# google-research/semivl

Measured on AMD Instinct MI355X. Metric: train images/sec (512^2, ViT-B/16), higher is better.
Workload: dtype f32 (fp32 in / out / accumulate everywhere; the MFMA products as split 16-bit terms with fp32 accumulation: the ViT's linears, in_proj weight gradients and fused attention and the decoder's 3x3 convolutions (tiled: forward, input and weight gradient; dilated: forward, input gradient) on fp16 x 2 ope; 1 GPU; SemiVL step, pascal N=21, vlm-vlg-aspp-s2p4-sk04-ftap-mcvitb, 512x512, bs=16/GPU labeled + 16/GPU unlabeled (BASELINE configs[1]); global_batch=32, parallelism=dp1

## Files before the change

### semivl_amd/csrc/gemm_planes_impl.h

```cpp
#pragma once
#include "svl_common.h"
#include "planes_split_h2.h"
#include <atomic>
#include <type_traits>

struct PlanesP {
  const char* A;
  const char* B;
  long a_ks, b_ks;
  const int* a_se;
  const int* b_se;
  const float* a_rn;
  const float* b_bd;
  int* p_se;
  int p_np;
  int epi_fast;
  int b_rb;
  int M, N, K;
  float* C;
  long ldc;
  char* P;
  long p_ks;
  const float* bias;
  int act;
  float* preact;
  const float* resid;
  long ldr;
  int accumulate;
  int tiles_n, full_m, tail_rows;
  int rcnt[8], fstart[8];
  int panel;
#ifdef SVL_X6P_TIMING
  unsigned long long* dbg;
#endif
};
#ifdef SVL_X6P_TIMING
#define X6P_STAMP(slot)                                                                      \
  do {                                                                                       \
    if (p.dbg && lane == 0 && (wave & 3) == 0) {                                             \
      p.dbg[((long)blockIdx.x * 2 + (wave >> 2)) * 8 + (slot)] = wall_clock64();            \
      p.dbg[((long)blockIdx.x * 2 + (wave >> 2)) * 8 + 4 + (slot)] = clock64();             \
    }                                                                                        \
  } while (0)
#else
#define X6P_STAMP(slot) do {} while (0)
#endif

namespace {

typedef __bf16 bf16x8 __attribute__((ext_vector_type(8)));
typedef int i32x4 __attribute__((ext_vector_type(4)));
typedef unsigned int u32x4 __attribute__((ext_vector_type(4)));

constexpr int BM = 256;
constexpr int CH = 1024;
constexpr int NSTAGE = 3;

template <int I, int N_, typename F>
__device__ __forceinline__ void static_for(F&& f) {
  if constexpr (I < N_) {
    f(std::integral_constant<int, I>{});
    static_for<I + 1, N_>(f);
  }
}

template <int NP> struct FragOf;
template <> struct FragOf<3> { typedef bf16x8 T; };
template <> struct FragOf<2> { typedef f16x8 T; };
template <int NP>
__device__ __forceinline__ f32x16 mfma16(const typename FragOf<NP>::T& x, const typename FragOf<NP>::T& y, const f32x16& c) {
  if constexpr (NP == 3) return __builtin_amdgcn_mfma_f32_32x32x16_bf16(x, y, c, 0, 0, 0);
  else return __builtin_amdgcn_mfma_f32_32x32x16_f16(x, y, c, 0, 0, 0);
}


__device__ __forceinline__ void glds16(const char* base_, unsigned lane_off, unsigned lds_dst_) {
  const unsigned long long bv = (unsigned long long)base_;
  const unsigned b_hi = (unsigned)__builtin_amdgcn_readfirstlane((int)(bv >> 32));
  const unsigned b_lo = (unsigned)__builtin_amdgcn_readfirstlane((int)(unsigned)bv);
  const char* base = (const char*)(((unsigned long long)b_hi << 32) | (unsigned long long)b_lo);
  const unsigned lds_dst = __builtin_amdgcn_readfirstlane(lds_dst_);
  unsigned keep;
  asm volatile("s_mov_b32 %0, m0\n\ts_mov_b32 m0, %3\n\ts_nop 3\n\tglobal_load_lds_dwordx4 %2, %1\n\ts_mov_b32 m0, %0"
               : "=&s"(keep)
               : "s"(base), "v"(lane_off), "s"(lds_dst)
               : "memory");
}

template <int N_>
__device__ __forceinline__ void wait_vm() {
  static_assert(N_ >= 0 && N_ < 64, "vmcnt");
  asm volatile("s_waitcnt vmcnt(%0)" ::"n"(N_) : "memory");
}

__device__ __forceinline__ void split3x8(const float (&x)[8], bf16x8& h0, bf16x8& h1, bf16x8& h2) {
#pragma unroll
  for (int j = 0; j < 8; ++j) {
    float v = x[j];
    h0[j] = (__bf16)v;
    v -= (float)h0[j];
    h1[j] = (__bf16)v;
    v -= (float)h1[j];
    h2[j] = (__bf16)v;
  }
}


struct TileRef { int m0, rows, tn; };
__device__ __forceinline__ TileRef tile_of_block(const PlanesP& p) {
  TileRef t;
  const int lin = (int)blockIdx.x, x = lin & 7, idx = lin >> 3;
  const int rc = p.rcnt[x];
  if (idx < rc) {
    t.m0 = p.full_m * BM;
    t.rows = p.tail_rows;
    t.tn = idx * 8 + x;
  } else {
    const int f = p.fstart[x] + idx - rc;
    const int gsz = p.full_m * p.panel;
    const int cg = f / gsz, r = f - cg * gsz;
    const int w = min(p.panel, p.tiles_n - cg * p.panel);
    const int tm = r / w;
    t.tn = cg * p.panel + (r - tm * w);
    t.m0 = tm * BM;
    t.rows = BM;
  }
  return t;
}

enum { EPI_LIGHT = 0, EPI_GELU = 1, EPI_DGELU = 2 };

template <int NP, int TM, int TN, int EPI>
__device__ __forceinline__ void x6p_epilogue(const PlanesP& p, f32x16 (&acc)[TM][TN], int m0, int mvalid, int wm, int nw,
                                             char* wl, int lane) {
  const int l31 = lane & 31, hi = lane >> 5;
  constexpr int WC = TN * 32;
  constexpr int RS = WC * 4 + 16;
  constexpr int LPR = WC / 4;
  static_assert((32 * LPR) % 64 == 0, "readback steps must be whole wave instructions");
  const bool vec = (p.ldc % 4 == 0) && (reinterpret_cast<uintptr_t>(p.C) % 16 == 0) &&
                   (reinterpret_cast<uintptr_t>(p.preact) % 16 == 0);
  const bool rvec = p.resid && (p.ldr % 4 == 0) && (reinterpret_cast<uintptr_t>(p.resid) % 16 == 0);

  auto store_rows = [&](float* dst, const f32x16 (&o)[TN], int mloc, bool accumulate) __attribute__((always_inline)) {
    static_for<0, TN>([&](auto J) {
      constexpr int j = decltype(J)::value;
      static_for<0, 4>([&](auto G) {
        constexpr int g = decltype(G)::value;
        f32x4 q = {o[j][4 * g], o[j][4 * g + 1], o[j][4 * g + 2], o[j][4 * g + 3]};
        *reinterpret_cast<f32x4*>(wl + l31 * RS + (j * 32 + 8 * g + 4 * hi) * 4) = q;
      });
    });
#pragma unroll
    for (int it = 0; it < 32 * LPR / 64; ++it) {
      const int idx = it * 64 + lane, row = idx / LPR, rc4 = (idx - row * LPR) * 4;
      const f32x4 q = *reinterpret_cast<const f32x4*>(wl + row * RS + rc4 * 4);
      const int n = nw + rc4;
      if (mloc + row < mvalid && n < p.N) {
        float* d = dst + (long)(m0 + mloc + row) * p.ldc + n;
        if (vec && n + 4 <= p.N) {
          f32x4 v = q;
          if (accumulate) v += *reinterpret_cast<const f32x4*>(d);
          *reinterpret_cast<f32x4*>(d) = v;
        } else {
#pragma unroll
          for (int e = 0; e < 4; ++e)
            if (n + e < p.N) d[e] = accumulate ? d[e] + q[e] : q[e];
        }
      }
    }
  };

  static_for<0, TM>([&](auto I) {
    constexpr int i = decltype(I)::value;
    const int mloc = (wm * TM + i) * 32;
    if (mloc < mvalid) {
      const int m = m0 + mloc + l31;
      const bool mok = mloc + l31 < mvalid;
      if constexpr (NP == 2) {
        const int ea = p.a_se ? p.a_se[m] : 0;
        static_for<0, TN>([&](auto J) {
          constexpr int j = decltype(J)::value;
          static_for<0, 4>([&](auto G) {
            constexpr int g = decltype(G)::value;
            const int n = nw + j * 32 + 8 * g + 4 * hi;
            i32x4 eb = {0, 0, 0, 0};
            if (p.b_se && n < p.N) eb = *reinterpret_cast<const i32x4*>(p.b_se + n);
#pragma unroll
            for (int e = 0; e < 4; ++e) acc[i][j][4 * g + e] = __builtin_amdgcn_ldexpf(acc[i][j][4 * g + e], ea + eb[e]);
          });
        });
      }
      if (p.bias) {
        static_for<0, TN>([&](auto J) {
          constexpr int j = decltype(J)::value;
          static_for<0, 4>([&](auto G) {
            constexpr int g = decltype(G)::value;
            const int n = nw + j * 32 + 8 * g + 4 * hi;
#pragma unroll
            for (int e = 0; e < 4; ++e) acc[i][j][4 * g + e] += n + e < p.N ? p.bias[n + e] : 0.f;
          });
        });
      }
      if (p.preact) store_rows(p.preact, acc[i], mloc, false);
      static_for<0, TN>([&](auto J) {
        constexpr int j = decltype(J)::value;
        static_for<0, 4>([&](auto G) {
          constexpr int g = decltype(G)::value;
          const int n = nw + j * 32 + 8 * g + 4 * hi;
          float rv[4] = {0.f, 0.f, 0.f, 0.f};
          if (p.resid && mok && n < p.N) {
            const float* rp = p.resid + (long)m * p.ldr + n;
            if (rvec && n + 4 <= p.N) {
              const f32x4 q = *reinterpret_cast<const f32x4*>(rp);
              rv[0] = q[0]; rv[1] = q[1]; rv[2] = q[2]; rv[3] = q[3];
            } else {
#pragma unroll
              for (int e = 0; e < 4; ++e) rv[e] = n + e < p.N ? rp[e] : 0.f;
            }
          }
#pragma unroll
          for (int e = 0; e < 4; ++e) {
            float v = acc[i][j][4 * g + e];
            if constexpr (EPI == EPI_GELU) v = gelu_erf(v) + rv[e];
            else if constexpr (EPI == EPI_DGELU) v *= gelu_erf_grad(rv[e]);
            else {
              if (p.act == SVL_ACT_RELU) v = fmaxf(v, 0.f);
              if (p.act == SVL_ACT_MUL_DRELU) v = rv[e] > 0.f ? v : 0.f;
              else v += rv[e];
            }
            acc[i][j][4 * g + e] = v;
          }
        });
      });
      if (p.C) store_rows(p.C, acc[i], mloc, p.accumulate != 0);
      if (p.P) {
        int eo = 0;
        if (p.p_np == 2) {
          float bound = p.a_rn[m] * p.b_bd[0] + p.b_bd[1];
          if constexpr (EPI == EPI_DGELU) bound *= 1.13f;
          eo = scale_exp_of(bound);
          if (nw == 0 && hi == 0) p.p_se[m] = eo;
        }
        static_for<0, TN>([&](auto J) {
          constexpr int j = decltype(J)::value;
          static_for<0, 2>([&](auto G2) {
            constexpr int g2 = decltype(G2)::value;
            const int nb = nw + j * 32 + 16 * g2;
            if (nb < p.N) {
              float o8[8];
#pragma unroll
              for (int e = 0; e < 8; ++e) o8[e] = acc[i][j][8 * g2 + e];
              if (p.p_np == 2) {
                f16x8 h0, h1;
                split2x8(o8, eo, h0, h1);
                char* q = p.P + (long)(nb >> 4) * p.p_ks + (long)((m0 + mloc) >> 5) * (2 * CH) + lane * 16;
                *reinterpret_cast<f16x8*>(q) = h0;
                *reinterpret_cast<f16x8*>(q + CH) = h1;
              } else {
                bf16x8 h0, h1, h2;
                split3x8(o8, h0, h1, h2);
                char* q = p.P + (long)(nb >> 4) * p.p_ks + (long)((m0 + mloc) >> 5) * (3 * CH) + lane * 16;
                *reinterpret_cast<bf16x8*>(q) = h0;
                *reinterpret_cast<bf16x8*>(q + CH) = h1;
                *reinterpret_cast<bf16x8*>(q + 2 * CH) = h2;
              }
            }
          });
        });
      }
    }
  });
}


template <int NP, int TM, int TN, int EPI>
__device__ __forceinline__ void x6p_epilogue_fast(const PlanesP& p, f32x16 (&acc)[TM][TN], int m0, int mvalid, int wm, int nw,
                                                  char* wl, int lane) {
  const int l31 = lane & 31, hi = lane >> 5;
  constexpr int WC = TN * 32, RS = WC * 4 + 16, LPR = WC / 4, NIT = 32 * LPR / 64;
  const int mw = m0 + wm * TM * 32;
  const int rows_w = mvalid - wm * TM * 32;
  float* lb = reinterpret_cast<float*>(wl + 32 * RS);
  int* le = reinterpret_cast<int*>(lb + WC);
#pragma unroll
  for (int c = lane; c < WC; c += 64) {
    const bool ok = nw + c < p.N;
    lb[c] = (p.bias && ok) ? p.bias[nw + c] : 0.f;
    if constexpr (NP == 2) le[c] = (p.b_se && ok) ? p.b_se[nw + c] : 0;
  }
  int ea[TM];
  static_for<0, TM>([&](auto I) { ea[decltype(I)::value] = (NP == 2 && p.a_se) ? p.a_se[mw + decltype(I)::value * 32 + l31] : 0; });
  int eo[TM];
  static_for<0, TM>([&](auto I) { eo[decltype(I)::value] = 0; });
  if (p.P && p.p_np == 2) {
    const float bd0 = p.b_bd[0], bd1 = p.b_bd[1];
    static_for<0, TM>([&](auto I) {
      constexpr int i = decltype(I)::value;
      float bound = p.a_rn[mw + i * 32 + l31] * bd0 + bd1;
      if constexpr (EPI == EPI_DGELU) bound *= 1.13f;
      eo[i] = scale_exp_of(bound);
    });
  }
  auto resid4 = [&](int i, int j, int g) __attribute__((always_inline)) {
    f32x4 r = {0.f, 0.f, 0.f, 0.f};
    const int n = nw + 4 * hi + j * 32 + 8 * g;
    if (i * 32 + l31 < rows_w && n < p.N) r = *reinterpret_cast<const f32x4*>(p.resid + (long)(mw + i * 32 + l31) * p.ldr + n);
    return r;
  };
  auto store_rows = [&](float* dst, const f32x16 (&o)[TN], int i, bool accumulate) __attribute__((always_inline)) {
    static_for<0, TN>([&](auto J) {
      constexpr int j = decltype(J)::value;
      static_for<0, 4>([&](auto G) {
        constexpr int g = decltype(G)::value;
        f32x4 q = {o[j][4 * g], o[j][4 * g + 1], o[j][4 * g + 2], o[j][4 * g + 3]};
        *reinterpret_cast<f32x4*>(wl + l31 * RS + (j * 32 + 8 * g + 4 * hi) * 4) = q;
      });
    });
    constexpr int HB = NIT > 4 ? 4 : NIT;
    static_for<0, NIT / HB>([&](auto H) {
      constexpr int h0 = decltype(H)::value * HB;
      f32x4 q[HB];
      float* d[HB];
      bool ok[HB];
#pragma unroll
      for (int it = 0; it < HB; ++it) {
        const int idx = (h0 + it) * 64 + lane, row = idx / LPR, c4 = (idx - row * LPR) * 4;
        q[it] = *reinterpret_cast<const f32x4*>(wl + row * RS + c4 * 4);
        d[it] = dst + (long)(mw + i * 32 + row) * p.ldc + nw + c4;
        ok[it] = nw + c4 < p.N && i * 32 + row < rows_w;
      }
      if (accumulate) {
#pragma unroll
        for (int it = 0; it < HB; ++it)
          if (ok[it]) q[it] += *reinterpret_cast<const f32x4*>(d[it]);
      }
#pragma unroll
      for (int it = 0; it < HB; ++it)
        if (ok[it]) *reinterpret_cast<f32x4*>(d[it]) = q[it];
    });
  };

  constexpr bool RES = EPI != EPI_GELU;
  f32x4 rv[TN][4];
  static_for<0, TN>([&](auto J) {
    static_for<0, 4>([&](auto G) {
      rv[decltype(J)::value][decltype(G)::value] = (RES && p.resid) ? resid4(0, decltype(J)::value, decltype(G)::value) : f32x4{0.f, 0.f, 0.f, 0.f};
    });
  });
  static_for<0, TM>([&](auto I) {
    constexpr int i = decltype(I)::value;
    if (i * 32 < rows_w) {
      __builtin_amdgcn_sched_barrier(0);
      static_for<0, TN>([&](auto J) {
        constexpr int j = decltype(J)::value;
        static_for<0, 4>([&](auto G) {
          constexpr int g = decltype(G)::value;
          const int c = j * 32 + 8 * g + 4 * hi;
          if constexpr (NP == 2) {
            const i32x4 eb = *reinterpret_cast<const i32x4*>(le + c);
#pragma unroll
            for (int e = 0; e < 4; ++e) acc[i][j][4 * g + e] = __builtin_amdgcn_ldexpf(acc[i][j][4 * g + e], ea[i] + eb[e]);
          }
          const f32x4 b4 = *reinterpret_cast<const f32x4*>(lb + c);
#pragma unroll
          for (int e = 0; e < 4; ++e) acc[i][j][4 * g + e] += b4[e];
        });
      });
      __builtin_amdgcn_sched_barrier(0);
      if (p.preact) store_rows(p.preact, acc[i], i, false);
      __builtin_amdgcn_sched_barrier(0);
      static_for<0, TN>([&](auto J) {
        constexpr int j = decltype(J)::value;
        static_for<0, 4>([&](auto G) {
          constexpr int g = decltype(G)::value;
          const f32x4 r4 = RES ? rv[j][g] : f32x4{0.f, 0.f, 0.f, 0.f};
          if constexpr (RES && i + 1 < TM) {
            if (p.resid) rv[j][g] = resid4(i + 1, j, g);
          }
#pragma unroll
          for (int e = 0; e < 4; ++e) {
            float v = acc[i][j][4 * g + e];
            const float r = r4[e];
            if constexpr (EPI == EPI_GELU) v = gelu_erf(v) + r;
            else if constexpr (EPI == EPI_DGELU) v *= gelu_erf_grad(r);
            else {
              if (p.act == SVL_ACT_RELU) v = fmaxf(v, 0.f);
              if (p.act == SVL_ACT_MUL_DRELU) v = r > 0.f ? v : 0.f;
              else v += r;
            }
            acc[i][j][4 * g + e] = v;
          }
          if constexpr (EPI == EPI_DGELU) __builtin_amdgcn_sched_barrier(0);
        });
      });
      __builtin_amdgcn_sched_barrier(0);
      if (p.C) store_rows(p.C, acc[i], i, p.accumulate != 0);
      __builtin_amdgcn_sched_barrier(0);
      if (p.P) {
        if (p.p_np == 2 && nw == 0 && hi == 0) p.p_se[mw + i * 32 + l31] = eo[i];
        static_for<0, TN>([&](auto J) {
          constexpr int j = decltype(J)::value;
          static_for<0, 2>([&](auto G2) {
            constexpr int g2 = decltype(G2)::value;
            const int nb = nw + j * 32 + 16 * g2;
            if (nb < p.N) {
              float o8[8];
#pragma unroll
              for (int e = 0; e < 8; ++e) o8[e] = acc[i][j][8 * g2 + e];
              if (p.p_np == 2) {
                f16x8 h0, h1;
                split2x8(o8, eo[i], h0, h1);
                char* q = p.P + (long)(nb >> 4) * p.p_ks + (long)((mw + i * 32) >> 5) * (2 * CH) + lane * 16;
                *reinterpret_cast<f16x8*>(q) = h0;
                *reinterpret_cast<f16x8*>(q + CH) = h1;
              } else {
                bf16x8 h0, h1, h2;
                split3x8(o8, h0, h1, h2);
                char* q = p.P + (long)(nb >> 4) * p.p_ks + (long)((mw + i * 32) >> 5) * (3 * CH) + lane * 16;
                *reinterpret_cast<bf16x8*>(q) = h0;
                *reinterpret_cast<bf16x8*>(q + CH) = h1;
                *reinterpret_cast<bf16x8*>(q + 2 * CH) = h2;
              }
            }
          });
        });
      }
    }
  });
}


template <int NP> constexpr int prod_a(int t) {
  return NP == 3 ? (t == 0 ? 2 : (t == 2 || t == 3) ? 1 : 0) : (t == 0 ? 1 : 0);
}
template <int NP> constexpr int prod_b(int t) {
  return NP == 3 ? (t == 1 ? 2 : (t == 2 || t == 4) ? 1 : 0) : (t == 1 ? 1 : 0);
}

template <int NP, int BN, int EPI, bool EF>
__global__ __launch_bounds__(512) void gemm_x6p_kernel(const PlanesP p) {
  extern __shared__ __attribute__((aligned(1024))) char sm[];
  constexpr int WN = BN == 192 ? 2 : 4, WM = 8 / WN;
  constexpr int TM = BM / 32 / WM, TN = BN / 32 / WN;
  constexpr int NCHA = BM / 32 * NP, NCHB = BN / 32 * NP, NCH = NCHA + NCHB;
  constexpr int STAGE = NCH * CH;
  constexpr int CPW = (NCH + 7) / 8;
  constexpr bool EVEN = NCH % 8 == 0;
  static_assert(NSTAGE * STAGE <= 160 * 1024 && 8 * (32 * (TN * 128 + 16) + TN * 32 * 8) <= 160 * 1024, "LDS");

  const int tid = threadIdx.x, lane = tid & 63, l31 = lane & 31, hi = lane >> 5;
  const int wave = __builtin_amdgcn_readfirstlane(tid >> 6);
  const int grp = wave >> 2, wm = wave / WN, wq = wave % WN;

  X6P_STAMP(0);
  const TileRef tr = tile_of_block(p);
  const int m0 = tr.m0, n0 = tr.tn * BN, mvalid = tr.rows;
  const int nblk = (mvalid + 31) >> 5;
  const int vb = min(TM, max(0, nblk - wm * TM));

  const char* a_src = p.A + (long)(m0 >> 5) * (NP * CH);
  const char* b_src = p.B + (long)tr.tn * (NCHB * CH);
  const unsigned lane16 = lane * 16;
  const unsigned sm_base = (unsigned)(uintptr_t)(__attribute__((address_space(3))) char*)sm;
  const int nk = p.K >> 4;

  auto issue = [&](int kg, int st) __attribute__((always_inline)) {
    const char* ak = a_src + (long)kg * p.a_ks;
    const char* bk = b_src + (long)kg * p.b_ks;
    const unsigned dst = sm_base + st * STAGE;
    static_for<0, CPW>([&](auto I) {
      constexpr int i = decltype(I)::value;
      const int c = wave + 8 * i;
      if (EVEN || i + 1 < CPW || c < NCH) {
        const char* s;
        if constexpr (8 * i + 7 < NCHA) {
          const int rb = c / NP;
          s = ak + (rb < nblk ? c : c - NP * rb) * CH;
        } else {
          static_assert(8 * i >= NCHA, "A / B chunk boundary must fall on a multiple of 8");
          const int cb = c - NCHA, rb = cb / NP;
          s = bk + (tr.tn * (BN / 32) + rb < p.b_rb ? cb : cb - NP * rb) * CH;
        }
        glds16(s, lane16, dst + c * CH);
      }
    });
  };
  const bool short_wave = !EVEN && wave >= NCH % 8;
  auto wait_older = [&]() __attribute__((always_inline)) {
    if constexpr (EVEN) wait_vm<CPW>();
    else {
      if (short_wave) wait_vm<CPW - 1>();
      else wait_vm<CPW>();
    }
  };

  f32x16 acc[TM][TN];
  static_for<0, TM>([&](auto I) {
    static_for<0, TN>([&](auto J) {
#pragma unroll
      for (int r = 0; r < 16; ++r) acc[decltype(I)::value][decltype(J)::value][r] = 0.f;
    });
  });

  const int fa = lane * 16 + wm * (TM * NP * CH);
  const int fb = lane * 16 + NCHA * CH + wq * (TN * NP * CH);

  issue(0, 0);
  if (nk > 1) {
    issue(1, 1);
    wait_older();
  } else {
    wait_vm<0>();
  }
  __builtin_amdgcn_s_barrier();
  X6P_STAMP(1);
  if (grp == 1) __builtin_amdgcn_s_barrier();
  __builtin_amdgcn_sched_barrier(0);

  constexpr int NPROD = NP == 3 ? 6 : 3;
  auto kloop = [&](auto FULLT) __attribute__((always_inline)) {
    constexpr bool FULL = decltype(FULLT)::value;
    typedef typename FragOf<NP>::T frag;
    frag a[NP][TM], b[NP][TN];
    int st = 0;
    for (int kg = 0; kg < nk; ++kg) {
      const char* S = sm + st * STAGE;
      {
        static_for<0, NP>([&](auto P) {
          constexpr int pl = decltype(P)::value;
          static_for<0, TN>([&](auto J) {
            b[pl][decltype(J)::value] = *reinterpret_cast<const frag*>(S + fb + (decltype(J)::value * NP + pl) * CH);
          });
        });
        static_for<0, NP>([&](auto P) {
          constexpr int pl = decltype(P)::value;
          static_for<0, TM>([&](auto I) {
            a[pl][decltype(I)::value] = *reinterpret_cast<const frag*>(S + fa + (decltype(I)::value * NP + pl) * CH);
          });
        });
      }
      if (kg + 2 < nk) {
        int st2 = st + 2;
        if (st2 >= NSTAGE) st2 -= NSTAGE;
        issue(kg + 2, st2);
        wait_older();
      } else {
        wait_vm<0>();
      }
      asm volatile("s_waitcnt lgkmcnt(0)" ::: "memory");
      __builtin_amdgcn_sched_barrier(0);
      __builtin_amdgcn_s_barrier();
      __builtin_amdgcn_sched_barrier(0);
      __builtin_amdgcn_s_setprio(1);
      if constexpr (FULL) {
        static_for<0, NPROD>([&](auto T) {
          constexpr int t = decltype(T)::value;
          constexpr int PA = prod_a<NP>(t), PB = prod_b<NP>(t);
          static_for<0, TM>([&](auto I) {
            static_for<0, TN>([&](auto J) {
              constexpr int i = decltype(I)::value, j = decltype(J)::value;
              acc[i][j] = mfma16<NP>(b[PB][j], a[PA][i], acc[i][j]);
            });
          });
        });
      } else {
        static_for<0, TM>([&](auto I) {
          constexpr int i = decltype(I)::value;
          if (i < vb) {
            static_for<0, NPROD>([&](auto T) {
              constexpr int t = decltype(T)::value;
              constexpr int PA = prod_a<NP>(t), PB = prod_b<NP>(t);
              static_for<0, TN>([&](auto J) {
                constexpr int j = decltype(J)::value;
                acc[i][j] = mfma16<NP>(b[PB][j], a[PA][i], acc[i][j]);
              });
            });
          }
        });
      }
      __builtin_amdgcn_s_setprio(0);
      __builtin_amdgcn_sched_barrier(0);
      __builtin_amdgcn_s_barrier();
      __builtin_amdgcn_sched_barrier(0);
      st = st + 1 == NSTAGE ? 0 : st + 1;
    }
  };
  if (vb == TM) kloop(std::true_type{});
  else kloop(std::false_type{});
  if (grp == 0) __builtin_amdgcn_s_barrier();
  X6P_STAMP(2);

  const int nw = n0 + wq * (TN * 32);
  char* wl = sm + wave * (32 * (TN * 128 + 16) + TN * 32 * 8);
  if constexpr (EF) x6p_epilogue_fast<NP, TM, TN, EPI>(p, acc, m0, mvalid, wm, nw, wl, lane);
  else x6p_epilogue<NP, TM, TN, EPI>(p, acc, m0, mvalid, wm, nw, wl, lane);
#ifdef SVL_X6P_TIMING
  asm volatile("s_waitcnt vmcnt(0)" ::: "memory");
#endif
  X6P_STAMP(3);
}


inline uint64_t attr_bit() {
  int dev = 0;
  (void)hipGetDevice(&dev);
  return 1ull << (dev & 63);
}
inline bool attr_needed(std::atomic<uint64_t>& mask) { return !(mask.load(std::memory_order_acquire) & attr_bit()); }

template <int NP, int BN, int EPI, bool EF>
int launch_kernel(const PlanesP& q, long blocks, hipStream_t st) {
  constexpr int TN_ = BN / 32 / (BN == 192 ? 2 : 4);
  constexpr size_t stages = (size_t)NSTAGE * ((BM + BN) / 32 * NP) * CH, scratch = (size_t)8 * (32 * (TN_ * 128 + 16) + TN_ * 32 * 8);
  constexpr size_t lds = stages > scratch ? stages : scratch;
  static std::atomic<uint64_t> mask{0};
  if (attr_needed(mask)) {
    SVL_HIP_CHECK(hipFuncSetAttribute(reinterpret_cast<const void*>(gemm_x6p_kernel<NP, BN, EPI, EF>),
                                      hipFuncAttributeMaxDynamicSharedMemorySize, (int)lds));
    mask.fetch_or(attr_bit(), std::memory_order_acq_rel);
  }
  hipLaunchKernelGGL((gemm_x6p_kernel<NP, BN, EPI, EF>), dim3((unsigned)blocks), dim3(512), lds, st, q);
  SVL_LAUNCH_CHECK("svl_gemm_planes_f32");
  return SVL_OK;
}

template <int NP, int BN, bool EF>
int launch_tile(PlanesP q, hipStream_t st) {
  q.tiles_n = (q.N + BN - 1) / BN;
  q.full_m = q.M / BM;
  q.tail_rows = q.M % BM;
  const long nf = (long)q.full_m * q.tiles_n, nr = q.tail_rows ? q.tiles_n : 0, total = nf + nr;
  if (total <= 0 || total > 0x7fffffffL) {
    svl_set_error("svl_gemm_planes_f32: bad tile count %ld", total);
    return SVL_ERR_INVALID_ARG;
  }
  const int pw = 6;
  q.panel = pw < q.tiles_n ? pw : q.tiles_n;
  long fs = 0;
  for (int x = 0; x < 8; ++x) {
    const long blocks = (total - x + 7) / 8, rag = nr > x ? (nr - x + 7) / 8 : 0;
    q.rcnt[x] = (int)rag;
    q.fstart[x] = (int)fs;
    fs += blocks - rag;
  }
  if (q.act == SVL_ACT_GELU) return launch_kernel<NP, BN, EPI_GELU, EF>(q, total, st);
  if (q.act == SVL_ACT_MUL_DGELU) return launch_kernel<NP, BN, EPI_DGELU, EF>(q, total, st);
  return launch_kernel<NP, BN, EPI_LIGHT, EF>(q, total, st);
}

template <int NP>
int launch(const PlanesP& q, hipStream_t st) {
  auto cost = [&](int bn) {
    const long tiles = (long)(q.M / BM) * ((q.N + bn - 1) / bn);
    const long rounds = tiles > 0 ? (tiles + 255) / 256 : 1;
    return (double)rounds * bn * (bn == 128 ? 1.15 : bn == 192 ? 1.04 : 1.0);
  };
  int bn = 0;
  {
    bn = 256;
    if (q.N <= 128) bn = 128;
    else {
      if (cost(192) < cost(bn)) bn = 192;
      if (cost(128) < cost(bn)) bn = 128;
    }
  }
  const bool al16 = ((reinterpret_cast<uintptr_t>(q.C) | reinterpret_cast<uintptr_t>(q.preact) | reinterpret_cast<uintptr_t>(q.resid)) & 15) == 0;
  const bool ef = q.epi_fast && al16 && (q.N & 3) == 0 && (q.ldc & 3) == 0 && (!q.resid || (q.ldr & 3) == 0) &&
                  !(q.act == SVL_ACT_GELU && q.resid);
  if (!ef) return launch_tile<NP, 128, false>(q, st);
  if (bn == 128) return launch_tile<NP, 128, true>(q, st);
  if (bn == 192) return launch_tile<NP, 192, true>(q, st);
  return launch_tile<NP, 256, true>(q, st);
}

}
```

Measured before the change: 105.4 images/s.

## Add dedicated strip kernel for small M-tail rows in planes GEMM

When the M dimension leaves a tail of at most 32 rows, a separate warp-specialized strip kernel handles it. Loader waves stream A/B chunks into an LDS ring while compute waves each own one 32-column strip, so the ragged tail no longer runs as full-size tiles in the main kernel. This cuts wasted MFMA work and LDS traffic on partial tiles, e.g. the CLS-token tail rows in ViT GEMMs. The cost is an extra kernel launch, plus a getenv call on every GEMM launch.

```diff
diff --git a/semivl_amd/csrc/gemm_planes_impl.h b/semivl_amd/csrc/gemm_planes_impl.h
--- a/semivl_amd/csrc/gemm_planes_impl.h
+++ b/semivl_amd/csrc/gemm_planes_impl.h
@@ -2,6 +2,7 @@
 #include "svl_common.h"
 #include "planes_split_h2.h"
 #include <atomic>
+#include <stdlib.h>
 #include <type_traits>
 
 struct PlanesP {
@@ -602,6 +603,138 @@
 }
 
 
+template <int NP, int SN>
+struct StripCfg {
+  static constexpr int KB = 4;
+  static constexpr int CK = (1 + SN) * NP;
+  static constexpr int STAGE = KB * CK * CH;
+  static constexpr int NS = 144 * 1024 / STAGE > 8 ? 8 : 144 * 1024 / STAGE;
+  static constexpr int VMW = (NS - 2) * CK;
+  static constexpr int THREADS = (KB + SN) * 64;
+  static constexpr int WL = 32 * (128 + 16) + 32 * 8;
+  static constexpr size_t LDS = (size_t)NS * STAGE;
+  static_assert(NS >= 3 && VMW < 64 && SN * WL <= NS * STAGE, "strip ring");
+};
+
+template <int NP, int SN, int EPI, bool EF>
+__global__ __launch_bounds__((4 + SN) * 64) void gemm_x6p_strip_kernel(const PlanesP p) {
+  extern __shared__ __attribute__((aligned(1024))) char sm[];
+  typedef StripCfg<NP, SN> Cfg;
+  constexpr int KB = Cfg::KB, CK = Cfg::CK, STAGE = Cfg::STAGE, NS = Cfg::NS;
+  const int tid = threadIdx.x, lane = tid & 63;
+  const int wave = __builtin_amdgcn_readfirstlane(tid >> 6);
+  const int nk = p.K >> 4, nb = (nk + KB - 1) / KB;
+  const int m0 = p.full_m * BM;
+  const int cb0 = (int)blockIdx.x * SN;
+  auto barrier = [&]() __attribute__((always_inline)) {
+    __builtin_amdgcn_sched_barrier(0);
+    __builtin_amdgcn_s_barrier();
+    __builtin_amdgcn_sched_barrier(0);
+  };
+
+  if (wave >= SN) {
+    const int l = wave - SN;
+    const char* a_src = p.A + (long)(m0 >> 5) * (NP * CH);
+    const unsigned lane16 = lane * 16;
+    const unsigned sm_base = (unsigned)(uintptr_t)(__attribute__((address_space(3))) char*)sm + l * (CK * CH);
+    auto issue = [&](int b, int st) __attribute__((always_inline)) {
+      const int kg = min(b * KB + l, nk - 1);
+      const char* ak = a_src + (long)kg * p.a_ks;
+      const char* bk = p.B + (long)kg * p.b_ks;
+      const unsigned dst = sm_base + st * STAGE;
+      static_for<0, NP>([&](auto P) { glds16(ak + decltype(P)::value * CH, lane16, dst + decltype(P)::value * CH); });
+      static_for<0, SN>([&](auto J) {
+        constexpr int j = decltype(J)::value;
+        const int cb = min(cb0 + j, p.b_rb - 1);
+        static_for<0, NP>([&](auto P) {
+          constexpr int pl = decltype(P)::value;
+          glds16(bk + (long)(cb * NP + pl) * CH, lane16, dst + (NP + j * NP + pl) * CH);
+        });
+      });
+    };
+    for (int b = 0; b < NS; ++b)
+      if (b < nb) issue(b, b);
+    if (nb >= NS) wait_vm<Cfg::VMW>();
+    else wait_vm<0>();
+    barrier();
+    barrier();
+    int st = 0;
+    for (int b = 0; b < nb; ++b) {
+      if (b + NS < nb) {
+        issue(b + NS, st);
+        wait_vm<Cfg::VMW>();
+      } else {
+        wait_vm<0>();
+      }
+      barrier();
+      st = st + 1 == NS ? 0 : st + 1;
+    }
+    return;
+  }
+
+  typedef typename FragOf<NP>::T frag;
+  constexpr int NPROD = NP == 3 ? 6 : 3;
+  f32x16 acc[1][1];
+#pragma unroll
+  for (int r = 0; r < 16; ++r) acc[0][0][r] = 0.f;
+  const char* fbase = sm + lane * 16;
+  const int fb = (NP + wave * NP) * CH;
+  constexpr int LGKM0 = 0xC07F;
+  frag fa[2][KB][NP], fbv[2][KB][NP];
+  auto load = [&](auto U, int st) __attribute__((always_inline)) {
+    constexpr int u = decltype(U)::value;
+    const char* S = fbase + st * STAGE;
+    static_for<0, KB>([&](auto G) {
+      constexpr int g = decltype(G)::value;
+      static_for<0, NP>([&](auto P) {
+        constexpr int pl = decltype(P)::value;
+        fa[u][g][pl] = *reinterpret_cast<const frag*>(S + g * (CK * CH) + pl * CH);
+        fbv[u][g][pl] = *reinterpret_cast<const frag*>(S + g * (CK * CH) + fb + pl * CH);
+      });
+    });
+  };
+  auto mm = [&](auto U, int cnt) __attribute__((always_inline)) {
+    constexpr int u = decltype(U)::value;
+    static_for<0, KB>([&](auto G) {
+      constexpr int g = decltype(G)::value;
+      if (g < cnt) {
+        static_for<0, NPROD>([&](auto T) {
+          constexpr int t = decltype(T)::value;
+          acc[0][0] = mfma16<NP>(fbv[u][g][prod_b<NP>(t)], fa[u][g][prod_a<NP>(t)], acc[0][0]);
+        });
+      }
+    });
+  };
+  auto step = [&](auto U, int b, int st_next) __attribute__((always_inline)) {
+    constexpr int u = decltype(U)::value;
+    load(std::integral_constant<int, 1 - u>{}, st_next);
+    __builtin_amdgcn_sched_barrier(0);
+    mm(U, min(KB, nk - b * KB));
+    __builtin_amdgcn_s_waitcnt(LGKM0);
+    barrier();
+  };
+  barrier();
+  load(std::integral_constant<int, 0>{}, 0);
+  __builtin_amdgcn_s_waitcnt(LGKM0);
+  barrier();
+  int st = 1;
+  for (int b = 0; b < nb; b += 2) {
+    step(std::integral_constant<int, 0>{}, b, st);
+    st = st + 1 == NS ? 0 : st + 1;
+    if (b + 1 < nb) {
+      step(std::integral_constant<int, 1>{}, b + 1, st);
+      st = st + 1 == NS ? 0 : st + 1;
+    }
+  }
+  const int nw = (cb0 + wave) * 32;
+  if (nw < p.N) {
+    char* wl = sm + wave * Cfg::WL;
+    if constexpr (EF) x6p_epilogue_fast<NP, 1, 1, EPI>(p, acc, m0, p.tail_rows, 0, nw, wl, lane);
+    else x6p_epilogue<NP, 1, 1, EPI>(p, acc, m0, p.tail_rows, 0, nw, wl, lane);
+  }
+}
+
+
 inline uint64_t attr_bit() {
   int dev = 0;
   (void)hipGetDevice(&dev);
@@ -625,11 +758,49 @@
   return SVL_OK;
 }
 
+template <int NP, int SN, int EPI, bool EF>
+int launch_strip_kernel(const PlanesP& q, hipStream_t st) {
+  typedef StripCfg<NP, SN> Cfg;
+  static std::atomic<uint64_t> mask{0};
+  if (attr_needed(mask)) {
+    SVL_HIP_CHECK(hipFuncSetAttribute(reinterpret_cast<const void*>(gemm_x6p_strip_kernel<NP, SN, EPI, EF>),
+                                      hipFuncAttributeMaxDynamicSharedMemorySize, (int)Cfg::LDS));
+    mask.fetch_or(attr_bit(), std::memory_order_acq_rel);
+  }
+  const int blocks = ((q.N + 31) / 32 + SN - 1) / SN;
+  hipLaunchKernelGGL((gemm_x6p_strip_kernel<NP, SN, EPI, EF>), dim3((unsigned)blocks), dim3(Cfg::THREADS), Cfg::LDS, st, q);
+  SVL_LAUNCH_CHECK("svl_gemm_planes_f32 (strip)");
+  return SVL_OK;
+}
+
+template <int NP, bool EF>
+int launch_strip(const PlanesP& q, hipStream_t st) {
+  const char* w = getenv("SVL_PLANES_STRIP_W");
+  if (w && atoi(w) == 64) {
+    if (q.act == SVL_ACT_GELU) return launch_strip_kernel<NP, 2, EPI_GELU, EF>(q, st);
+    if (q.act == SVL_ACT_MUL_DGELU) return launch_strip_kernel<NP, 2, EPI_DGELU, EF>(q, st);
+    return launch_strip_kernel<NP, 2, EPI_LIGHT, EF>(q, st);
+  }
+  if (q.act == SVL_ACT_GELU) return launch_strip_kernel<NP, 1, EPI_GELU, EF>(q, st);
+  if (q.act == SVL_ACT_MUL_DGELU) return launch_strip_kernel<NP, 1, EPI_DGELU, EF>(q, st);
+  return launch_strip_kernel<NP, 1, EPI_LIGHT, EF>(q, st);
+}
+
+constexpr int STRIP_MAX_ROWS = 32;
+
 template <int NP, int BN, bool EF>
 int launch_tile(PlanesP q, hipStream_t st) {
   q.tiles_n = (q.N + BN - 1) / BN;
   q.full_m = q.M / BM;
   q.tail_rows = q.M % BM;
+  if (q.tail_rows > 0 && q.tail_rows <= STRIP_MAX_ROWS) {
+    const char* off = getenv("SVL_PLANES_NO_STRIP");
+    if (!(off && atoi(off) != 0)) {
+      const int rc = launch_strip<NP, EF>(q, st);
+      if (rc != SVL_OK || q.full_m == 0) return rc;
+      q.tail_rows = 0;
+    }
+  }
   const long nf = (long)q.full_m * q.tiles_n, nr = q.tail_rows ? q.tiles_n : 0, total = nf + nr;
   if (total <= 0 || total > 0x7fffffffL) {
     svl_set_error("svl_gemm_planes_f32: bad tile count %ld", total);
```

New measurement: 104.9 images/s. No clear change (-0.5%).
